# christhetree/mod_extraction

Measured on AMD Instinct MI355X. Metric: 44.1 kHz audio-seconds/sec (train step), interwoven ph/fl/ch, higher is better.
Workload: dtype f32

## Files before the change

mod_extraction_amd/csrc/wgrad_kvec_f16.hip:

```cpp
#include "conv_common.h"
#include <stdlib.h>

typedef _Float16 half8 __attribute__((ext_vector_type(8)));
typedef _Float16 half4 __attribute__((ext_vector_type(4)));
typedef short short4v __attribute__((__vector_size__(4 * sizeof(short))));

#define WK_KS_MAX 6
#define WK_CH (WK_KS_MAX * 32)
#define WK_AP (WK_CH + 16)
#define WK_BR (WK_CH + 12)

#define WK_A_BYTES (2 * 64 * WK_AP * 2)
#define WK_B_ROWS ((WK_BR + 7) / 8 * 8)
#define WK_LDS_BYTES (WK_A_BYTES + 2 * WK_B_ROWS * 32)

struct WgradKvecArgs {
    const float *G;
    const unsigned char *amax;
    const float *scale;
    const _Float16 *xk_hi, *xk_lo;
    float *part;
    int B, H, Wv, rows_per_slab, n_slabs;
    int packed;
};

__device__ __forceinline__ floatx4 mfma_16x16x32(half8 a, half8 b, floatx4 c)
{
    return __builtin_amdgcn_mfma_f32_16x16x32_f16(a, b, c, 0, 0, 0);
}

__device__ __forceinline__ int wk_a_slot(int c8) { return c8 < 4 ? 8 * c8 : 8 * (c8 - 4) + 4; }
__device__ __forceinline__ half8 tr_frag16(const unsigned char *img, int lane_off, int r0)
{
    const unsigned char *ptr = img + lane_off + r0 * 32;
    const short4v v0 = __builtin_amdgcn_ds_read_tr16_b64_v4i16((short4v __attribute__((address_space(3))) *)ptr);
    const short4v v1 = __builtin_amdgcn_ds_read_tr16_b64_v4i16((short4v __attribute__((address_space(3))) *)(ptr + 16 * 32));
    typedef short short8v __attribute__((__vector_size__(8 * sizeof(short))));
    const short8v both = __builtin_shufflevector(v0, v1, 0, 1, 2, 3, 4, 5, 6, 7);
    return __builtin_bit_cast(half8, both);
}

__global__ __launch_bounds__(256, 2) void wgrad_kvec_f16_kernel(WgradKvecArgs a)
{
    extern __shared__ __attribute__((aligned(256))) unsigned char wk_smem[];
    _Float16 *const dzA = reinterpret_cast<_Float16 *>(wk_smem);
    _Float16 *const xB = reinterpret_cast<_Float16 *>(wk_smem + WK_A_BYTES);
    const int tid = threadIdx.x, lane = tid & 63, wave = __builtin_amdgcn_readfirstlane(tid >> 6);
    const int tap0 = wave * 3 + (wave >> 1);
    const int m16 = lane & 15, kg = lane >> 4;
    const int slab = blockIdx.x;
    const int Hp = a.H >> 1;
    const float S = a.scale[0];

    floatx4 acc[CV_KW];
#pragma unroll
    for (int i = 0; i < CV_KW; ++i) acc[i] = floatx4{0.f, 0.f, 0.f, 0.f};

    const int a_lane = (m16 * WK_AP + 8 * kg) * 2;
    const int b_lane = (4 * kg + (m16 >> 2)) * 32 + (m16 & 3) * 8;
    constexpr int A_SPLIT = 64 * WK_AP * 2, B_SPLIT = WK_B_ROWS * 32;
    const unsigned char *Ab = reinterpret_cast<const unsigned char *>(dzA);
    const unsigned char *Bb = reinterpret_cast<const unsigned char *>(xB);

    const int row_begin = slab * a.rows_per_slab;
    int row_end = row_begin + a.rows_per_slab;
    if (row_end > a.B * a.H) row_end = a.B * a.H;
    constexpr int NA = 64 * (WK_CH / 4) / 256, NB = (2 * WK_BR * 2 + 255) / 256;
    floatx4 ga[NA], vb[NB];
    unsigned ama[NA];
    auto issue_g = [&](int rid, int w0) {
        const int b = rid / a.H, h = rid - b * a.H;
        const int npos = (CV_PITCH - w0 >= WK_CH) ? WK_CH : (CV_PITCH - w0);
#pragma unroll
        for (int q = 0; q < NA; ++q) {
            const int i = tid + q * 256, co = i / (WK_CH / 4), c4 = i - co * (WK_CH / 4);
            ga[q] = floatx4{0.f, 0.f, 0.f, 0.f};
            ama[q] = 0x02020202u;
            if (c4 * 4 < npos) {
                const size_t off = (((size_t)b * 64 + co) * Hp + (h >> 1)) * CV_PITCH + w0 + c4 * 4;
                ga[q] = __builtin_nontemporal_load(reinterpret_cast<const floatx4 *>(a.G + off));
                ama[q] = __builtin_nontemporal_load(reinterpret_cast<const unsigned *>(a.amax + off));
            }
        }
    };
    auto issue_x = [&](int rid, int w0) {
        const int b = rid / a.H, h = rid - b * a.H;
        const int npos = (CV_PITCH - w0 >= WK_CH) ? WK_CH : (CV_PITCH - w0);
#pragma unroll
        for (int q = 0; q < NB; ++q) {
            const int i = tid + q * 256;
            const int split = i / (WK_BR * 2), k = i - split * (WK_BR * 2);
            const int pos = k >> 1, part = k & 1, w = w0 - 6 + pos;
            vb[q] = floatx4{0.f, 0.f, 0.f, 0.f};
            if (i < 2 * WK_BR * 2 && pos < npos + 12 && w >= 0 && w < CV_PITCH)
                vb[q] = *reinterpret_cast<const floatx4 *>((split ? a.xk_lo : a.xk_hi) +
                                                           (((size_t)b * a.H + h) * CV_PITCH + w) * 16 + part * 8);
        }
    };
    auto commit = [&](int rid, int w0) {
        const int h = rid % a.H;
        const unsigned want = (unsigned)(h & 1);
#pragma unroll
        for (int q = 0; q < NA; ++q) {
            const int i = tid + q * 256, co = i / (WK_CH / 4), c4 = i - co * (WK_CH / 4);
            const int wq = w0 + c4 * 4;
            half4 hi, lo;
            if (a.packed) {
                unsigned v[4];
#pragma unroll
                for (int e = 0; e < 4; ++e) v[e] = ((ama[q] >> (8 * e)) & 0xffu) == want ? __float_as_uint(ga[q][e]) : 0u;
                const unsigned h01 = __builtin_amdgcn_perm(v[1], v[0], 0x05040100u), h23 = __builtin_amdgcn_perm(v[3], v[2], 0x05040100u);
                const unsigned l01 = __builtin_amdgcn_perm(v[1], v[0], 0x07060302u), l23 = __builtin_amdgcn_perm(v[3], v[2], 0x07060302u);
                typedef unsigned uintx2 __attribute__((ext_vector_type(2)));
                hi = __builtin_bit_cast(half4, uintx2{h01, h23});
                lo = __builtin_bit_cast(half4, uintx2{l01, l23});
            } else {
#pragma unroll
            for (int e = 0; e < 4; ++e) {
                const bool keep = ((ama[q] >> (8 * e)) & 0xffu) == want && wq + e < a.Wv;
                const float v = keep ? ga[q][e] * S : 0.0f;
                const _Float16 hh = (_Float16)v;
                hi[e] = hh;
                lo[e] = (_Float16)(v - (float)hh);
            }
            }
            const int slot = (c4 >> 3) * 32 + wk_a_slot(c4 & 7);
            *reinterpret_cast<half4 *>(dzA + co * WK_AP + slot) = hi;
            *reinterpret_cast<half4 *>(dzA + 64 * WK_AP + co * WK_AP + slot) = lo;
        }
#pragma unroll
        for (int q = 0; q < NB; ++q) {
            const int i = tid + q * 256;
            if (i < 2 * WK_BR * 2) {
                const int split = i / (WK_BR * 2), k = i - split * (WK_BR * 2);
                *reinterpret_cast<floatx4 *>(xB + (size_t)split * (WK_B_ROWS * 16) + (k >> 1) * 16 + (k & 1) * 8) = vb[q];
            }
        }
    };

    int rid = row_begin, w0 = 0;
    if (rid < row_end) { issue_g(rid, w0); issue_x(rid, w0); }
    while (rid < row_end) {
        const int nks = (CV_PITCH - w0 >= WK_CH) ? WK_KS_MAX : (CV_PITCH - w0) / 32;
        int nrid, nw0 = w0;
        if (!(rid & 1)) nrid = rid + 1;
        else {
            nrid = rid - 1;
            nw0 = w0 + WK_CH;
            if (nw0 >= CV_PITCH) { nw0 = 0; nrid = rid + 1; }
        }
        __syncthreads();
        commit(rid, w0);
        if (nrid < row_end) {
            if (!(nrid & 1)) issue_g(nrid, nw0);
            issue_x(nrid, nw0);
        }
        __syncthreads();
        {
            {
#pragma unroll 1
            for (int ks = 0; ks < nks; ++ks) {
                half8 ah[5], al[5], bh[4], bl[4];
#pragma unroll
                for (int j = 0; j < 5; ++j) {
                    const int jt = j < 4 ? j : wave;
                    ah[j] = *reinterpret_cast<const half8 *>(Ab + a_lane + jt * (16 * WK_AP * 2) + ks * 64);
                    al[j] = *reinterpret_cast<const half8 *>(Ab + A_SPLIT + a_lane + jt * (16 * WK_AP * 2) + ks * 64);
                }
#pragma unroll
                for (int t = 0; t < 4; ++t) {
                    const int kw = t < 3 ? tap0 + t : 6;
                    bh[t] = tr_frag16(Bb, b_lane, ks * 32 + kw);
                    bl[t] = tr_frag16(Bb + B_SPLIT, b_lane, ks * 32 + kw);
                }
#pragma unroll
                for (int u = 0; u < 13; ++u) acc[u] = mfma_16x16x32(al[u < 12 ? (u & 3) : 4], bh[u < 12 ? (u >> 2) : 3], acc[u]);
#pragma unroll
                for (int u = 0; u < 13; ++u) acc[u] = mfma_16x16x32(ah[u < 12 ? (u & 3) : 4], bl[u < 12 ? (u >> 2) : 3], acc[u]);
#pragma unroll
                for (int u = 0; u < 13; ++u) acc[u] = mfma_16x16x32(ah[u < 12 ? (u & 3) : 4], bh[u < 12 ? (u >> 2) : 3], acc[u]);
            }
            }
        }
        rid = nrid;
        w0 = nw0;
    }
#pragma unroll
    for (int u = 0; u < CV_KW; ++u) {
        const int kw = u < 12 ? tap0 + (u >> 2) : 6, j = u < 12 ? (u & 3) : wave;
        float *dst = a.part + (((size_t)slab * CV_KW + kw) * 64 + j * 16) * 16;
#pragma unroll
        for (int r = 0; r < 4; ++r) dst[(4 * kg + r) * 16 + m16] = acc[u][r];
    }
}


__global__ __launch_bounds__(256) void wgrad_kvec_reduce_kernel(const float *__restrict__ part, int n_slabs,
                                                                const float *__restrict__ scale, float *__restrict__ dW)
{
    __shared__ double sh[16][17];
    const int total = CV_KW * 64 * 16;
    const int ol = threadIdx.x & 15, sl = threadIdx.x >> 4;
    const int j = blockIdx.x * 16 + ol;
    double s = 0.0;
    for (int i = sl; i < n_slabs; i += 16) s += (double)part[(size_t)i * total + j];
    sh[sl][ol] = s;
    __syncthreads();
    if (sl == 0) {
        double t = 0.0;
#pragma unroll
        for (int q = 0; q < 16; ++q) t += sh[q][ol];
        const int k = j & 15, co = (j >> 4) & 63, kw = j >> 10;
        if (k < 2 * CV_KH) {
            const int kh = k >> 1, ci = k & 1;
            dW[(((size_t)co * 2 + ci) * CV_KH + kh) * CV_KW + kw] = (float)(t * (double)scale[1]);
        }
    }
}

__global__ void wk_pow2_scale_kernel(const unsigned *__restrict__ amax_bits, float *__restrict__ scale)
{
    const float m = __uint_as_float(*amax_bits);
    int e = 0;
    if (m > 0.0f && m < 3.0e38f) {
        frexpf(m, &e);
        e = 10 - e;
        e = e > 100 ? 100 : (e < -100 ? -100 : e);
    }
    scale[0] = ldexpf(1.0f, e);
    scale[1] = ldexpf(1.0f, -e);
}

MX_EXPORT int mx_conv_block1_wgrad_f16(const float *G, const uint8_t *amax, const uint32_t *amax_bits, const void *xk_hi,
                                       const void *xk_lo, int64_t B, int64_t H, int64_t Wv, int64_t rows_per_slab,
                                       float *scale, float *part, float *dW, void *stream)
{
    if (!G || !amax || !amax_bits || !xk_hi || !xk_lo || !scale || !part || !dW || B <= 0 || rows_per_slab <= 0)
        return MX_ERR_ARG;
    if (H < 2 || (H & 1) || Wv <= 0 || Wv > CV_PITCH) return MX_ERR_UNSUPPORTED;
    rows_per_slab += rows_per_slab & 1;
    const int64_t n_slabs = (B * H + rows_per_slab - 1) / rows_per_slab;
    if (n_slabs > 1000000) return MX_ERR_UNSUPPORTED;
    hipStream_t st = (hipStream_t)stream;
    hipLaunchKernelGGL(wk_pow2_scale_kernel, dim3(1), dim3(1), 0, st, amax_bits, scale);
    WgradKvecArgs a{G, amax, scale, (const _Float16 *)xk_hi, (const _Float16 *)xk_lo, part, (int)B, (int)H, (int)Wv,
                    (int)rows_per_slab, (int)n_slabs, 0};
    static MxLdsLatch latch = {};
    if (mx_set_dyn_lds(latch, (const void *)wgrad_kvec_f16_kernel, WK_LDS_BYTES) != MX_OK) return MX_ERR_LAUNCH;
    hipLaunchKernelGGL(wgrad_kvec_f16_kernel, dim3((unsigned)n_slabs), dim3(256), WK_LDS_BYTES, st, a);
    const int total = CV_KW * 64 * 16;
    hipLaunchKernelGGL(wgrad_kvec_reduce_kernel, dim3(total / 16), dim3(256), 0, st, part, (int)n_slabs, scale, dW);
    return mx_launch_status();
}

MX_EXPORT int mx_conv_block1_wgrad_pair_f16(const void *Gp, const uint8_t *amax, const float *scale, const void *xk_hi,
                                            const void *xk_lo, int64_t B, int64_t H, int64_t Wv, int64_t rows_per_slab,
                                            float *part, float *dW, void *stream)
{
    if (!Gp || !amax || !scale || !xk_hi || !xk_lo || !part || !dW || B <= 0 || rows_per_slab <= 0) return MX_ERR_ARG;
    if (H < 2 || (H & 1) || Wv <= 0 || Wv > CV_PITCH) return MX_ERR_UNSUPPORTED;
    rows_per_slab += rows_per_slab & 1;
    const int64_t n_slabs = (B * H + rows_per_slab - 1) / rows_per_slab;
    if (n_slabs > 1000000) return MX_ERR_UNSUPPORTED;
    hipStream_t st = (hipStream_t)stream;
    WgradKvecArgs a{(const float *)Gp, amax, scale, (const _Float16 *)xk_hi, (const _Float16 *)xk_lo, part, (int)B, (int)H, (int)Wv,
                    (int)rows_per_slab, (int)n_slabs, 1};
    static MxLdsLatch latch = {};
    if (mx_set_dyn_lds(latch, (const void *)wgrad_kvec_f16_kernel, WK_LDS_BYTES) != MX_OK) return MX_ERR_LAUNCH;
    hipLaunchKernelGGL(wgrad_kvec_f16_kernel, dim3((unsigned)n_slabs), dim3(256), WK_LDS_BYTES, st, a);
    const int total = CV_KW * 64 * 16;
    hipLaunchKernelGGL(wgrad_kvec_reduce_kernel, dim3(total / 16), dim3(256), 0, st, part, (int)n_slabs, scale, dW);
    return mx_launch_status();
}
```

mod_extraction_amd/models.py:

```python
import logging
import math
import os
from typing import Dict, List, NamedTuple, Optional, Sequence, Tuple

import torch
from torch import Tensor as T, nn

from . import _hip

log = logging.getLogger(__name__)

CONV_PRECISION = os.environ.get("MODEX_CONV_PRECISION", "f16x3")
DEBUG_TAP = None
PITCH = 352
LN_EPS = 1e-5


def htk_mel_filterbank(n_freqs: int, f_min: float, f_max: float, n_mels: int, sample_rate: int) -> T:
    all_freqs = torch.linspace(0, sample_rate // 2, n_freqs)
    m_min = 2595.0 * math.log10(1.0 + (f_min / 700.0))
    m_max = 2595.0 * math.log10(1.0 + (f_max / 700.0))
    m_pts = torch.linspace(m_min, m_max, n_mels + 2)
    f_pts = 700.0 * (10.0 ** (m_pts / 2595.0) - 1.0)
    f_diff = f_pts[1:] - f_pts[:-1]
    slopes = f_pts.unsqueeze(0) - all_freqs.unsqueeze(1)
    down_slopes = (-1.0 * slopes[:, :-2]) / f_diff[:-1]
    up_slopes = slopes[:, 2:] / f_diff[1:]
    return torch.max(torch.zeros(1), torch.min(down_slopes, up_slopes))


def _band_limits(fb: T) -> Tuple[T, T]:
    nz = fb != 0
    any_nz = nz.any(dim=0)
    idx = torch.arange(fb.size(0)).unsqueeze(1).expand_as(fb)
    lo = torch.where(nz, idx, torch.full_like(idx, fb.size(0))).min(dim=0).values
    hi = torch.where(nz, idx + 1, torch.zeros_like(idx)).max(dim=0).values
    lo = torch.where(any_nz, lo, torch.zeros_like(lo))
    return lo.to(torch.int32), hi.to(torch.int32)


class _Buffers(nn.Module):
    """Plain namespace module (gives buffers their torchaudio state-dict key prefixes)."""


class MelSpectrogramHIP(nn.Module):

    def __init__(self, sample_rate: int, n_fft: int, hop_length: int, n_mels: int) -> None:
        super().__init__()
        if n_fft not in (512, 1024, 2048):
            raise NotImplementedError("mx_logmel_fwd is built for n_fft in {512, 1024, 2048}")
        self.sample_rate, self.n_fft, self.hop_length, self.n_mels = sample_rate, n_fft, hop_length, n_mels
        self.spectrogram = _Buffers()
        self.spectrogram.register_buffer("window", torch.hann_window(n_fft))
        self.mel_scale = _Buffers()
        self.mel_scale.register_buffer("fb", htk_mel_filterbank(n_fft // 2 + 1, 0.0, float(sample_rate // 2),
                                                                n_mels, sample_rate))
        k = torch.arange(n_fft, dtype=torch.float64) * (-2.0 * math.pi / n_fft)
        self.register_buffer("twiddle", torch.stack([torch.cos(k), torch.sin(k)], dim=1).float(), persistent=False)
        self._bands: Optional[Tuple[T, T, int]] = None

    def bands(self) -> Tuple[T, T]:
        fb = self.mel_scale.fb
        if self._bands is None or self._bands[2] != fb._version or self._bands[0].device != fb.device:
            lo, hi = _band_limits(fb.detach().cpu())
            self._bands = (lo.to(fb.device), hi.to(fb.device), fb._version)
        return self._bands[0], self._bands[1]

    def log_mel(self, x: T, n_frames: int, eps: float, masks: Sequence[int] = (0, 0, 0, 0), pitch: int = PITCH) -> T:
        B, C, N = x.shape
        xc = x.contiguous().float()
        out = torch.empty((B, C, self.n_mels, pitch), device=x.device, dtype=torch.float32)
        lo, hi = self.bands()
        f0, f1, t0, t1 = (int(v) for v in masks)
        _hip.call("mx_logmel_fwd", _hip.ptr(xc), B * C, N, _hip.ptr(self.spectrogram.window), _hip.ptr(self.twiddle),
                  _hip.ptr(self.mel_scale.fb), _hip.ptr(lo), _hip.ptr(hi), self.n_fft, self.hop_length, self.n_mels,
                  n_frames, pitch, float(eps), f0, f1, t0, t1, _hip.ptr(out), _hip.stream())
        return out


def specaugment_bounds(size: int, mask_param: int) -> Tuple[int, int]:
    value = torch.rand(1) * mask_param
    min_value = torch.rand(1) * (size - value)
    start = int(min_value.long())
    return start, start + int(value.long())


BLOCK1_F16 = os.environ.get("MODEX_BLOCK1", "f16x3") != "f32"
WGRAD_SPARSE = os.environ.get("MODEX_WGRAD", "sparse") != "dense"
WGRAD_SPARSE_MAX_T = int(os.environ.get("MODEX_WGRAD_SP_MAXT", "4"))
DGRAD_SPARSE = os.environ.get("MODEX_DGRAD", "sparse") != "dense"
DIRECT_GRADS = os.environ.get("MODEX_DIRECT_GRADS", "1") != "0"
STATS_FUSED = os.environ.get("MODEX_STATS", "fused") != "sweep"
GPOOL_FUSED = os.environ.get("MODEX_GPOOL", "fused") != "split"
LN_FUSED = os.environ.get("MODEX_LN", "fused") != "sweep"
BLOCK1_PAIR = os.environ.get("MODEX_BLOCK1_PAIR", "1") != "0"

KH, KW, TAPS, CO = 5, 13, 65, 64
W_F16_ELEMS = 4 * KH * KW * CO * 16
W_KVEC_ELEMS = KW * 2 * CO * 8
W_SP_ELEMS = 4 * 3 * 2 * KW * 2 * 64 * 16
KVEC_PART_ELEMS = KW * CO * 16
WS_ROW_KS = 22


def _wgrad_part(n_slabs: int, cin: int, dev) -> T:
    return torch.empty(n_slabs * TAPS * CO * cin, device=dev, dtype=torch.float32)


def _slabs(rows: int, n_target: int) -> Tuple[int, int]:
    rps = max(1, -(-rows // n_target))
    return rps, -(-rows // rps)


def _f16_pair(dev, *shape: int) -> Tuple[T, T]:
    return (torch.empty(shape, device=dev, dtype=torch.float16), torch.empty(shape, device=dev, dtype=torch.float16))


def _f32(dev, *shape: int) -> T:
    return torch.empty(shape, device=dev, dtype=torch.float32)


def _pack(w: T, flip: int) -> T:
    out = _f32(w.device, w.numel())
    _hip.call("mx_conv_pack_weights", _hip.ptr(w.contiguous()), w.size(0), w.size(1), flip, _hip.ptr(out),
              _hip.stream())
    return out


def _pack_f16(w: T, flip: int) -> Tuple[T, T]:
    hi, lo = _f16_pair(w.device, W_F16_ELEMS)
    _hip.call("mx_conv_pack_weights_f16", _hip.ptr(w.contiguous()), flip, _hip.ptr(hi), _hip.ptr(lo), _hip.stream())
    return hi, lo


def _reduce_rows(part: T, rows: int, cols: int, out: Optional[T] = None) -> T:
    if out is None:
        out = _f32(part.device, cols)
    _hip.call("mx_reduce_rows", _hip.ptr(part), rows, cols, 0, _hip.ptr(out), _hip.stream())
    return out


def _direct_grad_views(params) -> Optional[List[T]]:
    views = []
    base = None
    for p in params:
        if not (p.is_leaf and p.requires_grad):
            return None
        g = p.grad
        if g is None or not g.is_contiguous() or g._base is None or g.dtype != torch.float32:
            return None
        if base is None:
            base = g._base
        elif g._base is not base:
            return None
        views.append(g)
    if base is None or not getattr(base, "_modex_fresh", False):
        return None
    base._modex_fresh = False
    return views


class BlockRoute(NamedTuple):
    fwd: str
    stats: str
    leaves_stats: bool
    g_in: str
    operand: Optional[str]
    wgrad: str
    routed_pair: bool
    dgrad: Optional[str]
    ln_bwd: Optional[str]

    @property
    def dgrad_sparse(self) -> bool:
        return self.dgrad in ("sparse", "sparse+ln")


def plan_stack(cin0: int, dilations: Sequence[int], precision: str, n_frames: int,
               operands_kept: bool = True) -> Tuple[BlockRoute, ...]:
    n = len(dilations)
    fits = n_frames <= PITCH - 1
    blocks = []
    for l, t in enumerate(int(t) for t in dilations):
        if precision == "f16x3" and (cin0 if l == 0 else CO) == 64:
            sp_w = WGRAD_SPARSE and t <= WGRAD_SPARSE_MAX_T and fits
            sp_d = DGRAD_SPARSE and fits
            dgrad = ("sparse+ln" if LN_FUSED else "sparse") if sp_d else "dense"
            blocks.append(dict(fwd="f16x3", operand="kept" if operands_kept else "rederived", wgrad="sparse" if sp_w else "dense",
                               routed_pair=not sp_w or (l > 0 and not sp_d), dgrad=dgrad if l > 0 else None))
        elif precision == "f16x3" and l == 0 and cin0 == 2 and BLOCK1_F16 and t == 1:
            blocks.append(dict(fwd="kvec", operand=None, wgrad="f32", routed_pair=False, dgrad=None))
        else:
            blocks.append(dict(fwd="f32", operand=None, wgrad="f32", routed_pair=False, dgrad="f32" if l > 0 else None))
    for l, b in enumerate(blocks):
        b["stats"] = "epilogue" if l > 0 and blocks[l - 1]["leaves_stats"] else "sweep"
        b["leaves_stats"] = STATS_FUSED and l + 1 < n and b["fwd"] != "f32"
    blocks[-1]["g_in"] = "f32+gmax" if blocks[-1]["fwd"] == "f16x3" else "f32"
    kvec_kept = blocks[0]["fwd"] == "kvec" and operands_kept
    for l in range(n - 1, 0, -1):
        b, below = blocks[l], blocks[l - 1]
        pooled_only = l > 1 and below["wgrad"] == "sparse" and below["dgrad"] in ("sparse", "sparse+ln")
        if b["dgrad"] == "sparse+ln" and GPOOL_FUSED and pooled_only:
            b["ln_bwd"], below["g_in"] = "gpool", "pooled"
        elif b["dgrad"] == "sparse+ln" and BLOCK1_PAIR and l == 1 and kvec_kept:
            b["ln_bwd"], below["g_in"] = "pair", "pair"
        elif below["fwd"] == "f16x3" or (l == 1 and kvec_kept):
            b["ln_bwd"], below["g_in"] = "plain+gmax", "f32+gmax"
        else:
            b["ln_bwd"], below["g_in"] = "plain", "f32"
    blocks[0]["ln_bwd"] = None
    if kvec_kept and blocks[0]["g_in"] != "f32":
        blocks[0].update(operand="kept", wgrad="kvec_pair" if blocks[0]["g_in"] == "pair" else "kvec_scaled")
    return tuple(BlockRoute(**b) for b in blocks)


class _Act(NamedTuple):
    p: T
    slope: Optional[T] = None
    bias: Optional[T] = None
    stats_part: Optional[T] = None


class _Grad(NamedTuple):
    G: Optional[T] = None
    gmax: Optional[T] = None
    pooled: Optional[tuple] = None
    pair_scale: Optional[T] = None
    bsum: Optional[T] = None


class _Split(NamedTuple):
    G: Optional[T] = None
    dz: Tuple[Optional[T], Optional[T]] = (None, None)
    gc: Tuple[Optional[T], ...] = (None, None, None)
    scale: Optional[T] = None
    x16: Tuple[Optional[T], Optional[T]] = (None, None)


class _ParamGrads:

    def __init__(self, n: int, direct: Optional[List[T]]) -> None:
        self.direct, self.grads = direct, [None] * n

    def weight(self, i: int, w: T) -> T:
        self.grads[i] = self.direct[i] if self.direct is not None else torch.empty_like(w)
        return self.grads[i]

    def reduce(self, i: int, part: T, rows: int, cols: int) -> None:
        self.grads[i] = _reduce_rows(part, rows, cols, self.direct[i].view(-1) if self.direct is not None else None)

    def for_autograd(self) -> List[Optional[T]]:
        return [None] * len(self.grads) if self.direct is not None else self.grads


def _block_fwd(r: BlockRoute, x: _Act, w: T, b: T, a: T, n_frames: int, t: int, first: bool):
    B, cin, H, _ = x.p.shape
    dev, st = x.p.device, _hip.stream()
    stats = _f32(dev, B, cin, 2)
    if r.stats == "epilogue":
        _hip.call("mx_plane_stats_finish", _hip.ptr(x.stats_part), _hip.ptr(x.bias), _hip.ptr(x.slope), B, cin, H,
                  n_frames, LN_EPS, _hip.ptr(stats), st)
    else:
        _hip.call("mx_plane_stats", _hip.ptr(x.p), _hip.ptr(x.slope), B, cin, H, n_frames, LN_EPS, _hip.ptr(stats), st)
    a_out = a.contiguous()
    p = _f32(dev, B, 64, H // 2, PITCH)
    amax = torch.empty((B, 64, H // 2, PITCH), device=dev, dtype=torch.uint8)
    stats_part = _f32(dev, B, H // 2, 64, 2) if r.leaves_stats else None
    operand = None
    if r.fwd == "f16x3":
        operand = _f16_pair(dev, B, H, 4, PITCH, 16)
        _hip.call("mx_conv_prep_fwd_f16", _hip.ptr(x.p), _hip.ptr(stats), _hip.ptr(x.slope), B, H, n_frames,
                  _hip.ptr(operand[0]), _hip.ptr(operand[1]), st)
        w_hi, w_lo = _pack_f16(w, 0)
        _hip.call("mx_conv_block_fwd_f16", _hip.ptr(operand[0]), _hip.ptr(operand[1]), _hip.ptr(w_hi), _hip.ptr(w_lo),
                  _hip.ptr(b.contiguous()), B, H, n_frames, t, _hip.ptr(p), _hip.ptr(amax),
                  _hip.ptr(a_out) if r.leaves_stats else None, _hip.ptr(stats_part), st)
    elif r.fwd == "kvec":
        operand = _f16_pair(dev, B, H, 1, PITCH, 16)
        _hip.call("mx_conv_prep_fwd_kvec_f16", _hip.ptr(x.p), _hip.ptr(stats), B, H, n_frames, _hip.ptr(operand[0]),
                  _hip.ptr(operand[1]), st)
        wk_hi, wk_lo = _f16_pair(dev, W_KVEC_ELEMS)
        _hip.call("mx_conv_pack_weights_kvec_f16", _hip.ptr(w.detach().contiguous()), _hip.ptr(wk_hi), _hip.ptr(wk_lo), st)
        _hip.call("mx_conv_block1_fwd_f16", _hip.ptr(operand[0]), _hip.ptr(operand[1]), _hip.ptr(wk_hi), _hip.ptr(wk_lo),
                  _hip.ptr(b.contiguous()), B, H, n_frames, _hip.ptr(p), _hip.ptr(amax),
                  _hip.ptr(a_out) if r.leaves_stats else None, _hip.ptr(stats_part), st)
    else:
        wt = _pack(w, 0)
        _hip.call("mx_conv_block_fwd", _hip.ptr(x.p), _hip.ptr(stats), _hip.ptr(x.slope), _hip.ptr(wt),
                  _hip.ptr(b.contiguous()), B, cin, H, n_frames, t, 1 if first else 0, _hip.ptr(p), _hip.ptr(amax), st)
    return _Act(p, a_out, b.contiguous(), stats_part), (x.p, stats, amax), operand


def _head_bwd(r_last: BlockRoute, p_last: T, slope_last: T, wout: T, latent: T, out: T, d_out: T, d_latent: Optional[T],
              n_frames: int, gmax_cell: T, pg: _ParamGrads, i_wout: int, i_slope: int) -> _Grad:
    B, L, Hl, dev = out.size(0), out.size(1), p_last.size(2), out.device
    G = torch.empty_like(p_last)
    dw_part, db_part, ds_part = _f32(dev, B, L * 64), _f32(dev, B, L), _f32(dev, B, 64)
    gmax = gmax_cell if r_last.g_in == "f32+gmax" else None
    _hip.call("mx_head_bwd", _hip.ptr(p_last), _hip.ptr(slope_last), _hip.ptr(wout.contiguous()),
              _hip.ptr(latent), _hip.ptr(out), _hip.ptr(d_out), _hip.ptr(d_latent), B, 64, Hl, n_frames, L,
              _hip.ptr(G), _hip.ptr(dw_part), _hip.ptr(db_part), _hip.ptr(ds_part), _hip.ptr(gmax), _hip.stream())
    pg.reduce(i_wout, dw_part, B, L * 64)
    pg.grads[i_wout] = pg.grads[i_wout].view_as(wout)
    pg.reduce(i_wout + 1, db_part, B, L)
    pg.reduce(i_slope, ds_part, B, 64)
    return _Grad(G=G, gmax=gmax)


def _wgrad_f16x3(r: BlockRoute, l: int, g: _Grad, kept: dict, x_in: T, stats: T, amax: T, slope_prev: Optional[T],
                 n_frames: int, t: int, dW: T) -> _Split:
    B, _, H, _ = x_in.shape
    Hp, dev, st = H // 2, x_in.device, _hip.stream()
    dz = _f16_pair(dev, B, H, 4, PITCH, 16) if r.routed_pair else (None, None)
    if r.g_in == "pooled":
        gc_hi, gc_lo, gc_idx, gidx, scale = g.pooled
    else:
        ready = r.g_in == "f32+gmax"
        ws = g.gmax if ready else torch.empty(1, device=dev, dtype=torch.int32)
        scale = _f32(dev, 2)
        _hip.call("mx_conv_prep_dgrad_f16", _hip.ptr(g.G), _hip.ptr(amax), B, H, n_frames, _hip.ptr(ws),
                  1 if ready else 0, _hip.ptr(scale), _hip.ptr(dz[0]), _hip.ptr(dz[1]), st)
        gc_hi = gc_lo = gc_idx = gidx = None
        if r.wgrad == "sparse" or r.dgrad_sparse:
            gc_hi, gc_lo = _f16_pair(dev, B, Hp, 4, PITCH, 16)
            gc_idx = torch.empty((B, Hp, 4, PITCH), device=dev, dtype=torch.int32)
            if r.wgrad == "sparse":
                gidx = torch.empty((B, 64, Hp, WS_ROW_KS, 2), device=dev, dtype=torch.int16)
            _hip.call("mx_conv_prep_gpool_cl_f16", _hip.ptr(g.G), _hip.ptr(amax), _hip.ptr(scale), B, H, n_frames,
                      _hip.ptr(gc_hi), _hip.ptr(gc_lo), _hip.ptr(gc_idx), _hip.ptr(gidx), st)
    if r.operand == "kept":
        x_hi, x_lo = kept.pop(l)
    else:
        x_hi, x_lo = _f16_pair(dev, B, H, 4, PITCH, 16)
        _hip.call("mx_conv_prep_fwd_f16", _hip.ptr(x_in), _hip.ptr(stats), _hip.ptr(slope_prev), B, H, n_frames,
                  _hip.ptr(x_hi), _hip.ptr(x_lo), st)
    rps, n_slabs = _slabs(B * Hp if r.wgrad == "sparse" else B * H, 256)
    part = _wgrad_part(n_slabs, 64, dev)
    if r.wgrad == "sparse":
        _hip.call("mx_conv_block_wgrad_sp_f16", _hip.ptr(gc_hi), _hip.ptr(gc_lo), _hip.ptr(gidx), _hip.ptr(x_hi),
                  _hip.ptr(x_lo), _hip.ptr(scale), B, H, n_frames, t, rps, _hip.ptr(part), _hip.ptr(dW), st)
    else:
        _hip.call("mx_conv_block_wgrad_f16", _hip.ptr(dz[0]), _hip.ptr(dz[1]), _hip.ptr(x_hi), _hip.ptr(x_lo),
                  _hip.ptr(scale), B, H, t, rps, _hip.ptr(part), _hip.ptr(dW), st)
    return _Split(dz=dz if r.dgrad == "dense" else (None, None), gc=(gc_hi, gc_lo, gc_idx), scale=scale,
                  x16=(x_hi, x_lo) if r.dgrad == "sparse+ln" else (None, None))


def _weight_grad(r: BlockRoute, l: int, g: _Grad, kept: dict, x_in: T, stats: T, amax: T, slope_prev: Optional[T],
                 n_frames: int, t: int, dW: T) -> _Split:
    if r.fwd == "f16x3":
        return _wgrad_f16x3(r, l, g, kept, x_in, stats, amax, slope_prev, n_frames, t, dW)
    B, cin, H, _ = x_in.shape
    dev, st = x_in.device, _hip.stream()
    if r.wgrad in ("kvec_pair", "kvec_scaled"):
        xk_hi, xk_lo = kept.pop(l)
        rps, n_slabs = _slabs(B * H, 2048)
        part = _f32(dev, n_slabs * KVEC_PART_ELEMS)
        if r.wgrad == "kvec_pair":
            _hip.call("mx_conv_block1_wgrad_pair_f16", _hip.ptr(g.G), _hip.ptr(amax), _hip.ptr(g.pair_scale), _hip.ptr(xk_hi),
                      _hip.ptr(xk_lo), B, H, n_frames, rps, _hip.ptr(part), _hip.ptr(dW), st)
        else:
            scale1 = _f32(dev, 2)
            _hip.call("mx_conv_block1_wgrad_f16", _hip.ptr(g.G), _hip.ptr(amax), _hip.ptr(g.gmax), _hip.ptr(xk_hi),
                      _hip.ptr(xk_lo), B, H, n_frames, rps, _hip.ptr(scale1), _hip.ptr(part), _hip.ptr(dW), st)
    else:
        rps, n_slabs = _slabs(B * H, 256 if cin == 64 else 1024)
        part = _wgrad_part(n_slabs, cin, dev)
        _hip.call("mx_conv_block_wgrad", _hip.ptr(g.G), _hip.ptr(amax), _hip.ptr(x_in), _hip.ptr(stats),
                  _hip.ptr(slope_prev), B, cin, H, n_frames, t, rps, _hip.ptr(part), _hip.ptr(dW), st)
    return _Split(G=g.G)


def _data_grad(r: BlockRoute, l: int, d: _Split, w: T, amax: T, B: int, H: int, n_frames: int, t: int, zws: T):
    dev, st = w.device, _hip.stream()
    dxhat = _f32(dev, B, 64, H, PITCH)
    ln_part = gx_bits = None
    if r.dgrad_sparse:
        ws_hi, ws_lo = _f16_pair(dev, W_SP_ELEMS)
        _hip.call("mx_conv_pack_weights_sp_f16", _hip.ptr(w.detach().contiguous()), _hip.ptr(ws_hi), _hip.ptr(ws_lo), st)
        if r.dgrad == "sparse+ln":
            ln_part = _f32(dev, B, 64, H, 2, 2)
            gx_bits = zws[4 * l:4 * l + 2] if r.ln_bwd in ("gpool", "pair") else None
        _hip.call("mx_conv_block_dgrad_sp_f16", _hip.ptr(d.gc[0]), _hip.ptr(d.gc[1]), _hip.ptr(d.gc[2]),
                  _hip.ptr(ws_hi), _hip.ptr(ws_lo), _hip.ptr(d.scale), B, H, n_frames, t,
                  _hip.ptr(dxhat), _hip.ptr(d.x16[0]), _hip.ptr(d.x16[1]), _hip.ptr(ln_part), _hip.ptr(gx_bits), st)
    elif r.dgrad == "dense":
        w_hi, w_lo = _pack_f16(w, 1)
        _hip.call("mx_conv_block_dgrad_f16", _hip.ptr(d.dz[0]), _hip.ptr(d.dz[1]), _hip.ptr(w_hi), _hip.ptr(w_lo),
                  _hip.ptr(d.scale), B, H, n_frames, t, _hip.ptr(dxhat), st)
    else:
        wt_f = _pack(w, 1)
        _hip.call("mx_conv_block_dgrad", _hip.ptr(d.G), _hip.ptr(amax), _hip.ptr(wt_f), B, H, n_frames, t, _hip.ptr(dxhat), st)
    if DEBUG_TAP is not None:
        DEBUG_TAP[f"dxhat{l}"] = dxhat.clone()
    return dxhat, ln_part, gx_bits


def _ln_prelu_bwd(r: BlockRoute, l: int, x_in: T, dxhat: T, ln_part: Optional[T], gx_bits: Optional[T], stats: T,
                  slope_prev: T, amax_below: T, n_frames: int, zws: T) -> Tuple[_Grad, T]:
    B, _, H, _ = x_in.shape
    dev, st = x_in.device, _hip.stream()
    ds_part, bsum = _f32(dev, B, 64), _f32(dev, B, 64)
    if r.ln_bwd in ("gpool", "pair"):
        m12, scale_n = _f32(dev, B, 64, 2), _f32(dev, 2)
        bound_ws = torch.empty(1, device=dev, dtype=torch.int32)
        _hip.call("mx_ln_bwd_finish", _hip.ptr(ln_part), _hip.ptr(stats), _hip.ptr(slope_prev), _hip.ptr(gx_bits),
                  B, 64, H, n_frames, _hip.ptr(m12), _hip.ptr(bound_ws), _hip.ptr(scale_n), st)
    if r.ln_bwd == "gpool":
        gn_hi, gn_lo = _f16_pair(dev, B, H, 4, PITCH, 16)
        gn_idx = torch.empty((B, H, 4, PITCH), device=dev, dtype=torch.int32)
        gn_pidx = torch.empty((B, 64, H, WS_ROW_KS, 2), device=dev, dtype=torch.int16)
        part2 = _f32(dev, B, 64, H, 6, 2)
        _hip.call("mx_ln_prelu_bwd_gpool_f16", _hip.ptr(x_in), _hip.ptr(dxhat), _hip.ptr(amax_below),
                  _hip.ptr(stats), _hip.ptr(slope_prev), _hip.ptr(m12), _hip.ptr(scale_n), B, H, n_frames,
                  _hip.ptr(gn_hi), _hip.ptr(gn_lo), _hip.ptr(gn_idx), _hip.ptr(gn_pidx), _hip.ptr(part2),
                  _hip.ptr(ds_part), _hip.ptr(bsum), st)
        return _Grad(pooled=(gn_hi, gn_lo, gn_idx, gn_pidx, scale_n), bsum=bsum), ds_part
    if r.ln_bwd == "pair":
        _hip.call("mx_ln_prelu_bwd_pair", _hip.ptr(x_in), _hip.ptr(dxhat), _hip.ptr(stats), _hip.ptr(slope_prev),
                  B, 64, H, n_frames, _hip.ptr(ds_part), _hip.ptr(bsum), _hip.ptr(ln_part), _hip.ptr(scale_n), st)
        return _Grad(G=dxhat, pair_scale=scale_n, bsum=bsum), ds_part
    gmax = zws[4 * l + 2:4 * l + 3] if r.ln_bwd == "plain+gmax" else None
    _hip.call("mx_ln_prelu_bwd", _hip.ptr(x_in), _hip.ptr(dxhat), _hip.ptr(stats), _hip.ptr(slope_prev),
              B, 64, H, n_frames, _hip.ptr(ds_part), _hip.ptr(bsum), _hip.ptr(gmax), _hip.ptr(ln_part), st)
    return _Grad(G=dxhat, gmax=gmax, bsum=bsum), ds_part


class _CNNStack(torch.autograd.Function):

    @staticmethod
    def forward(ctx, logmel: T, n_frames: int, dilations: Tuple[int, ...], precision: str, *params: T):
        n_blocks = len(dilations)
        routes = plan_stack(logmel.size(1), dilations, precision, n_frames)
        keep = any(ctx.needs_input_grad)
        ctx.operands = {}
        x, saved = _Act(logmel), []
        for l, r in enumerate(routes):
            x, for_bwd, operand = _block_fwd(r, x, *params[3 * l:3 * l + 3], n_frames, int(dilations[l]), l == 0)
            saved += for_bwd
            if keep and r.operand == "kept":
                ctx.operands[l] = operand
            del operand
        wout, bout = params[3 * n_blocks], params[3 * n_blocks + 1]
        B, H, L, dev = logmel.size(0), x.p.size(2), wout.size(0), logmel.device
        latent, out = _f32(dev, B, 64, n_frames), _f32(dev, B, L, n_frames)
        _hip.call("mx_head_fwd", _hip.ptr(x.p), _hip.ptr(x.slope), _hip.ptr(wout.contiguous()),
                  _hip.ptr(bout.contiguous()), B, 64, H, n_frames, L, _hip.ptr(latent), _hip.ptr(out), _hip.stream())
        ctx.save_for_backward(*saved, x.p, latent, out, *params)
        ctx.param_objs = params
        ctx.meta = (n_frames, tuple(dilations), n_blocks, precision)
        return out, latent

    @staticmethod
    def backward(ctx, d_out: Optional[T], d_latent: Optional[T]):
        n_frames, dilations, n_blocks, precision = ctx.meta
        tensors = ctx.saved_tensors
        saved, (p_last, latent, out), params = tensors[:3 * n_blocks], tensors[3 * n_blocks:3 * n_blocks + 3], \
            tensors[3 * n_blocks + 3:]
        kept, ctx.operands = ctx.operands, None
        routes = plan_stack(saved[0].size(1), dilations, precision, n_frames, operands_kept=kept is not None)
        B, dev = out.size(0), out.device
        pg = _ParamGrads(len(params), _direct_grad_views(ctx.param_objs) if DIRECT_GRADS else None)
        d_out = (d_out if d_out is not None else torch.zeros_like(out)).contiguous()
        d_latent = d_latent.contiguous() if d_latent is not None else None
        zws = torch.zeros(4 * (n_blocks + 1), device=dev, dtype=torch.int32)
        g = _head_bwd(routes[-1], p_last, params[3 * (n_blocks - 1) + 2].contiguous(), params[3 * n_blocks], latent, out,
                      d_out, d_latent, n_frames, zws[4 * n_blocks:4 * n_blocks + 1], pg, 3 * n_blocks, 3 * (n_blocks - 1) + 2)
        for l in range(n_blocks - 1, -1, -1):
            r, t = routes[l], int(dilations[l])
            x_in, stats, amax = saved[3 * l:3 * l + 3]
            H = x_in.size(2)
            slope_prev = params[3 * (l - 1) + 2].contiguous() if l > 0 else None
            if DEBUG_TAP is not None:
                if r.g_in in ("f32", "f32+gmax"):
                    DEBUG_TAP[f"G{l}"] = g.G.clone()
                DEBUG_TAP[f"amax{l}"] = amax.clone()
                DEBUG_TAP[f"p{l}"] = (p_last if l == n_blocks - 1 else saved[3 * (l + 1)]).clone()
            bsum = g.bsum
            if bsum is None:
                bsum = _f32(dev, B, 64)
                _hip.call("mx_plane_sum", _hip.ptr(g.G), B * 64, H // 2, n_frames, _hip.ptr(bsum), _hip.stream())
            pg.reduce(3 * l + 1, bsum, B, 64)
            d = _weight_grad(r, l, g, kept, x_in, stats, amax, slope_prev, n_frames, t, pg.weight(3 * l, params[3 * l]))
            del g, bsum
            if l == 0:
                break
            dxhat, ln_part, gx_bits = _data_grad(r, l, d, params[3 * l], amax, B, H, n_frames, t, zws)
            del d
            g, ds_part = _ln_prelu_bwd(r, l, x_in, dxhat, ln_part, gx_bits, stats, slope_prev, saved[3 * (l - 1) + 2],
                                       n_frames, zws)
            del dxhat, ln_part
            pg.reduce(3 * (l - 1) + 2, ds_part, B, 64)
        return (None, None, None, None, *pg.for_autograd())


class Spectral2DCNN(nn.Module):
    def __init__(self,
                 in_ch: int = 1,
                 n_samples: int = 88200,
                 sr: float = 44100,
                 n_fft: int = 1024,
                 hop_len: int = 256,
                 n_mels: int = 256,
                 kernel_size: Tuple[int, int] = (5, 13),
                 out_channels: Optional[List[int]] = None,
                 bin_dilations: Optional[List[int]] = None,
                 temp_dilations: Optional[List[int]] = None,
                 pool_size: Tuple[int, int] = (3, 1),
                 latent_dim: int = 1,
                 freq_mask_amount: float = 0.0,
                 time_mask_amount: float = 0.0,
                 use_ln: bool = True,
                 eps: float = 1e-7) -> None:
        super().__init__()
        if out_channels is None:
            out_channels = [64] * 5
        if bin_dilations is None:
            bin_dilations = [1] * len(out_channels)
        if temp_dilations is None:
            temp_dilations = [2 ** idx for idx in range(len(out_channels))]
        assert len(out_channels) == len(bin_dilations) == len(temp_dilations)
        assert pool_size[1] == 1
        self.sr, self.n_fft, self.hop_len, self.n_mels = sr, n_fft, hop_len, n_mels
        self.kernel_size, self.pool_size, self.latent_dim = tuple(kernel_size), tuple(pool_size), latent_dim
        self.freq_mask_amount, self.time_mask_amount = freq_mask_amount, time_mask_amount
        self.use_ln, self.eps = use_ln, eps
        self.out_channels, self.bin_dilations, self.temp_dilations = list(out_channels), list(bin_dilations), \
            list(temp_dilations)
        self.in_ch = in_ch
        self.n_frames = n_samples // hop_len + 1
        self.generic = (self.kernel_size != (5, 13) or self.pool_size != (2, 1) or not use_ln
                        or any(c != 64 for c in out_channels) or any(d != 1 for d in bin_dilations)
                        or any(d not in (1, 2, 4, 8, 16) for d in temp_dilations) or in_ch not in (1, 2)
                        or self.n_frames > PITCH or n_mels % (2 ** len(out_channels)) != 0 or latent_dim > 4)
        if self.generic:
            n_bins = n_mels
            for _ in out_channels:
                n_bins //= self.pool_size[0]
            if n_bins < 1 or min(self.kernel_size) < 1 or min(self.bin_dilations + self.temp_dilations) < 1 or self.pool_size[0] > 255:
                raise ValueError(f"Spectral2DCNN: {n_mels} mel bins do not survive {len(out_channels)} poolings by "
                                 f"{self.pool_size[0]} (or a kernel size / dilation below 1)")
        self.conv_precision = CONV_PRECISION
        self.spectrogram = MelSpectrogramHIP(int(sr), n_fft, hop_len, n_mels)
        self.freq_mask_param = int(freq_mask_amount * n_mels)
        self.time_mask_param = int(time_mask_amount * self.n_frames)
        layers: List[nn.Module] = []
        n_bins, c_in = n_mels, in_ch
        for out_ch, b_dil, t_dil in zip(out_channels, bin_dilations, temp_dilations):
            if use_ln:
                layers.append(nn.LayerNorm([n_bins, self.n_frames], elementwise_affine=False))
            layers.append(nn.Conv2d(c_in, out_ch, self.kernel_size, stride=(1, 1), dilation=(b_dil, t_dil),
                                    padding="same"))
            layers.append(nn.MaxPool2d(kernel_size=self.pool_size))
            layers.append(nn.PReLU(num_parameters=out_ch))
            c_in, n_bins = out_ch, n_bins // self.pool_size[0]
        self.cnn = nn.Sequential(*layers)
        self.output = nn.Conv1d(out_channels[-1], latent_dim, kernel_size=(1,))

    def _stack_params(self) -> List[T]:
        ps: List[T] = []
        per, first = (4, 1) if self.use_ln else (3, 0)
        for i in range(len(self.out_channels)):
            conv, prelu = self.cnn[per * i + first], self.cnn[per * i + first + 2]
            w = conv.weight
            if i == 0 and self.in_ch == 1 and not self.generic:
                w = torch.cat([w, torch.zeros_like(w)], dim=1)
            ps += [w, conv.bias, prelu.weight]
        ps += [self.output.weight, self.output.bias]
        return ps

    def draw_masks(self) -> Tuple[int, int, int, int]:
        f0 = f1 = t0 = t1 = 0
        if self.training:
            if self.freq_mask_amount > 0:
                f0, f1 = specaugment_bounds(self.n_mels, self.freq_mask_param)
            if self.time_mask_amount > 0:
                t0, t1 = specaugment_bounds(self.n_frames, self.time_mask_param)
        return f0, f1, t0, t1

    def log_mel(self, x: T, masks: Optional[Sequence[int]] = None) -> T:
        assert x.ndim == 3
        n_frames = x.size(-1) // self.hop_len + 1
        assert n_frames == self.n_frames, "clip length does not match the LayerNorm shape"
        masks = self.draw_masks() if masks is None else masks
        if self.generic:
            with torch.no_grad():
                return self.spectrogram.log_mel(x, self.n_frames, self.eps, masks, pitch=self.n_frames)
        if self.in_ch == 1:
            x = torch.cat([x, torch.zeros_like(x)], dim=1)
        with torch.no_grad():
            return self.spectrogram.log_mel(x, self.n_frames, self.eps, masks)

    def forward(self, x: T, masks: Optional[Sequence[int]] = None) -> (T, T):
        logmel = self.log_mel(x, masks)
        if self.generic:
            from .cnn_generic import GenericCNNStack
            cfg = (self.kernel_size, int(self.pool_size[0]), bool(self.use_ln),
                   tuple(zip(self.out_channels, self.bin_dilations, self.temp_dilations)))
            return GenericCNNStack.apply(logmel, cfg, *self._stack_params())
        out, latent = _CNNStack.apply(logmel, self.n_frames, tuple(self.temp_dilations), self.conv_precision,
                                      *self._stack_params())
        return out, latent


class RandomLFO(nn.Module):

    def __init__(self,
                 n_samples: int,
                 sr: float,
                 use_shape_gt: bool = False,
                 use_phase_gt: bool = False,
                 use_freq_gt: bool = False,
                 shapes: Optional[List[str]] = None,
                 freq_min: float = 0.5,
                 freq_max: float = 3.0,
                 phase_error: float = 0.0,
                 freq_error: float = 0.0) -> None:
        super().__init__()
        self.n_samples, self.sr = n_samples, sr
        self.use_shape_gt, self.use_phase_gt, self.use_freq_gt = use_shape_gt, use_phase_gt, use_freq_gt
        self.shapes, self.freq_min, self.freq_max = shapes, freq_min, freq_max
        self.phase_error, self.freq_error = phase_error, freq_error

    def forward(self, batch_size: int, fx_params: Optional[Dict[str, T]] = None) -> T:
        from .modulations import make_rand_mod_signal
        shapes_gt = phase_gt = freq_gt = None
        if self.use_shape_gt:
            assert fx_params is not None and "shape" in fx_params
            shapes_gt = fx_params["shape"]
        if self.use_phase_gt:
            assert fx_params is not None and "phase" in fx_params
            phase_gt = fx_params["phase"]
        if self.use_freq_gt:
            assert fx_params is not None and "rate_hz" in fx_params
            freq_gt = fx_params["rate_hz"]
        return make_rand_mod_signal(batch_size, self.n_samples, self.sr, self.freq_min, self.freq_max, shapes_gt,
                                    self.shapes, phase_gt, self.phase_error, freq_gt, self.freq_error).unsqueeze(1)


class SpectrogramHIP(nn.Module):

    def __init__(self, n_fft: int, hop_length: int) -> None:
        super().__init__()
        if n_fft not in (512, 1024, 2048):
            raise NotImplementedError("mx_logmel_fwd is built for n_fft in {512, 1024, 2048}")
        self.n_fft, self.hop_length, self.n_bins = n_fft, hop_length, n_fft // 2 + 1
        self.register_buffer("window", torch.hann_window(n_fft))
        k = torch.arange(n_fft, dtype=torch.float64) * (-2.0 * math.pi / n_fft)
        self.register_buffer("twiddle", torch.stack([torch.cos(k), torch.sin(k)], dim=1).float(), persistent=False)
        self.register_buffer("eye", torch.eye(self.n_bins), persistent=False)
        self.register_buffer("band_lo", torch.arange(self.n_bins, dtype=torch.int32), persistent=False)
        self.register_buffer("band_hi", torch.arange(1, self.n_bins + 1, dtype=torch.int32), persistent=False)

    def log_power(self, x: T, n_frames: int, eps: float) -> T:
        assert x.ndim == 3 and x.size(1) == 1
        B, _, N = x.shape
        xc = x.contiguous().float()
        out = torch.empty((B, self.n_bins, PITCH), device=x.device, dtype=torch.float32)
        _hip.call("mx_logmel_fwd", _hip.ptr(xc), B, N, _hip.ptr(self.window), _hip.ptr(self.twiddle), _hip.ptr(self.eye),
                  _hip.ptr(self.band_lo), _hip.ptr(self.band_hi), self.n_fft, self.hop_length, self.n_bins, n_frames, PITCH,
                  float(eps), 0, 0, 0, 0, _hip.ptr(out), _hip.stream())
        return out

# ... 227 lines not shown
```

Before: 7635.

## Add 2:4 structured-sparse SMFMAC kernel for block-1 paired weight gradient

Adds a new block-1 weight-gradient kernel that exploits the 2:4 sparsity pattern implied by max-pool amax indices. It packs the pooled gradient into compressed halves plus nibble indices in LDS and uses smfmac 16x16x64 instructions, halving the MFMA work and reading the pooled G directly. The host signals sparse vs dense via the parity of rows_per_slab, which is an opaque encoding, and the new kernel uses a smaller channel chunk and different LDS layout.

```diff
diff --git a/mod_extraction_amd/csrc/wgrad_kvec_f16.hip b/mod_extraction_amd/csrc/wgrad_kvec_f16.hip
--- a/mod_extraction_amd/csrc/wgrad_kvec_f16.hip
+++ b/mod_extraction_amd/csrc/wgrad_kvec_f16.hip
@@ -180,6 +180,175 @@
 #pragma unroll
                 for (int u = 0; u < 13; ++u) acc[u] = mfma_16x16x32(ah[u < 12 ? (u & 3) : 4], bh[u < 12 ? (u >> 2) : 3], acc[u]);
             }
+            }
+        }
+        rid = nrid;
+        w0 = nw0;
+    }
+#pragma unroll
+    for (int u = 0; u < CV_KW; ++u) {
+        const int kw = u < 12 ? tap0 + (u >> 2) : 6, j = u < 12 ? (u & 3) : wave;
+        float *dst = a.part + (((size_t)slab * CV_KW + kw) * 64 + j * 16) * 16;
+#pragma unroll
+        for (int r = 0; r < 4; ++r) dst[(4 * kg + r) * 16 + m16] = acc[u][r];
+    }
+}
+
+typedef _Float16 half16 __attribute__((ext_vector_type(16)));
+#define WS_KS 4
+#define WS_CH (WS_KS * 32)
+#define WS_AP (WS_CH + 16)
+#define WS_BR (WS_CH + 12)
+#define WS_BROWS (WS_BR + 2)
+#define WS_BPAR (WS_BROWS * 32)
+#define WS_BSPLIT (2 * WS_BPAR)
+#define WS_A_BYTES (2 * 64 * WS_AP * 2)
+#define WS_LDS_BYTES (WS_A_BYTES + 2 * WS_BSPLIT)
+#define WS_IX_OFF (WS_CH * 2)
+
+__device__ __forceinline__ half16 tr_frag_sp(const unsigned char *img, int lane_off, int r0)
+{
+    typedef short4v __attribute__((address_space(3))) * lds4;
+    const unsigned char *ptr = img + lane_off + r0 * 32;
+    const short4v v0 = __builtin_amdgcn_ds_read_tr16_b64_v4i16((lds4)ptr);
+    const short4v v1 = __builtin_amdgcn_ds_read_tr16_b64_v4i16((lds4)(ptr + 2 * 32));
+    const short4v v2 = __builtin_amdgcn_ds_read_tr16_b64_v4i16((lds4)(ptr + 16 * 32));
+    const short4v v3 = __builtin_amdgcn_ds_read_tr16_b64_v4i16((lds4)(ptr + 18 * 32));
+    typedef short short8v __attribute__((__vector_size__(8 * sizeof(short))));
+    typedef short short16v __attribute__((__vector_size__(16 * sizeof(short))));
+    const short8v a = __builtin_shufflevector(v0, v1, 0, 1, 2, 3, 4, 5, 6, 7), b = __builtin_shufflevector(v2, v3, 0, 1, 2, 3, 4, 5, 6, 7);
+    const short16v all = __builtin_shufflevector(a, b, 0, 1, 2, 3, 4, 5, 6, 7, 8, 9, 10, 11, 12, 13, 14, 15);
+    return __builtin_bit_cast(half16, all);
+}
+
+__global__ __launch_bounds__(256, 2) void wgrad_kvec_sp_f16_kernel(WgradKvecArgs a)
+{
+    extern __shared__ __attribute__((aligned(256))) unsigned char wk_smem[];
+    _Float16 *const dzA = reinterpret_cast<_Float16 *>(wk_smem);
+    unsigned char *const xB = wk_smem + WS_A_BYTES;
+    const int tid = threadIdx.x, lane = tid & 63, wave = __builtin_amdgcn_readfirstlane(tid >> 6);
+    const int tap0 = wave * 3 + (wave >> 1);
+    const int m16 = lane & 15, kg = lane >> 4;
+    const int slab = blockIdx.x;
+    const int Hp = a.H >> 1;
+
+    floatx4 acc[CV_KW];
+#pragma unroll
+    for (int i = 0; i < CV_KW; ++i) acc[i] = floatx4{0.f, 0.f, 0.f, 0.f};
+
+    constexpr int A_SPLIT = 64 * WS_AP * 2, A_TILE = 16 * WS_AP * 2;
+    const int a_lane = (m16 * WS_AP + 8 * kg) * 2;
+    const int i_lane = m16 * WS_AP * 2 + WS_IX_OFF + 2 * kg;
+    const int b_lane = ((m16 >> 3) & 1) * WS_BPAR + (4 * kg + ((m16 >> 2) & 1)) * 32 + (m16 & 3) * 8;
+    const unsigned char *Ab = reinterpret_cast<const unsigned char *>(dzA);
+    const unsigned char *Bb = xB;
+
+    const int row_begin = slab * a.rows_per_slab;
+    int row_end = row_begin + a.rows_per_slab;
+    if (row_end > a.B * a.H) row_end = a.B * a.H;
+    constexpr int NA = 64 * (WS_CH / 4) / 256, NB = 5;
+    static_assert(WS_BR * 2 == 256 + 24, "the B staging deals 256 + 24 items per image");
+    const int t_par = lane >= 24, t_k = 256 + lane - 24 * t_par;
+    floatx4 vb[NB];
+    typedef unsigned uintx4 __attribute__((ext_vector_type(4)));
+    uintx4 ga[NA];
+    unsigned ama[NA];
+    auto issue = [&](int rid, int w0) {
+        const int b = rid / a.H, h = rid - b * a.H;
+        const int npos = (CV_PITCH - w0 >= WS_CH) ? WS_CH : (CV_PITCH - w0);
+#pragma unroll
+        for (int q = 0; q < NA; ++q) {
+            const int i = tid + q * 256, co = i / (WS_CH / 4), c4 = i - co * (WS_CH / 4);
+            ga[q] = uintx4{0u, 0u, 0u, 0u};
+            ama[q] = 0x02020202u;
+            if (c4 * 4 < npos) {
+                const size_t off = (((size_t)b * 64 + co) * Hp + (h >> 1)) * CV_PITCH + w0 + c4 * 4;
+                ga[q] = __builtin_nontemporal_load(reinterpret_cast<const uintx4 *>(a.G + off));
+                ama[q] = __builtin_nontemporal_load(reinterpret_cast<const unsigned *>(a.amax + off));
+            }
+        }
+        const long xoff = (((long)b * a.H + h) * CV_PITCH + w0 - 6) * 16;
+#pragma unroll
+        for (int img = 0; img < 4; ++img) {
+            const _Float16 *src = ((img >> 1) ? a.xk_lo : a.xk_hi) + xoff + (img & 1) * (CV_PITCH * 16);
+            const int pos = tid >> 1, w = w0 - 6 + pos;
+            vb[img] = floatx4{0.f, 0.f, 0.f, 0.f};
+            if (pos < npos + 12 && w >= 0 && w < CV_PITCH) vb[img] = *reinterpret_cast<const floatx4 *>(src + tid * 8);
+        }
+        vb[4] = floatx4{0.f, 0.f, 0.f, 0.f};
+        if (wave < 2 && lane < 48) {
+            const _Float16 *src = (wave ? a.xk_lo : a.xk_hi) + xoff + t_par * (CV_PITCH * 16);
+            const int pos = t_k >> 1, w = w0 - 6 + pos;
+            if (pos < npos + 12 && w >= 0 && w < CV_PITCH) vb[4] = *reinterpret_cast<const floatx4 *>(src + t_k * 8);
+        }
+    };
+    auto commit = [&]() {
+#pragma unroll
+        for (int q = 0; q < NA; ++q) {
+            const int i = tid + q * 256, co = i / (WS_CH / 4), c4 = i - co * (WS_CH / 4);
+            unsigned first[2], second[2], nib = 0;
+#pragma unroll
+            for (int c = 0; c < 2; ++c) {
+                const unsigned a0 = (ama[q] >> (16 * c)) & 0xffu, a1 = (ama[q] >> (16 * c + 8)) & 0xffu;
+                const unsigned x0 = a0 < 2u ? ga[q][2 * c] : 0u, x1 = a1 < 2u ? ga[q][2 * c + 1] : 0u;
+                const unsigned sel = (a0 & 1u) + 2u * (a1 & 1u);
+                const bool swap = sel == 1u;
+                first[c] = swap ? x1 : x0;
+                second[c] = swap ? x0 : x1;
+                nib |= ((0xEC94u >> (4 * sel)) & 0xfu) << (4 * c);
+            }
+            const unsigned h01 = __builtin_amdgcn_perm(second[0], first[0], 0x05040100u), h23 = __builtin_amdgcn_perm(second[1], first[1], 0x05040100u);
+            const unsigned l01 = __builtin_amdgcn_perm(second[0], first[0], 0x07060302u), l23 = __builtin_amdgcn_perm(second[1], first[1], 0x07060302u);
+            typedef unsigned uintx2 __attribute__((ext_vector_type(2)));
+            *reinterpret_cast<uintx2 *>(dzA + co * WS_AP + c4 * 4) = uintx2{h01, h23};
+            *reinterpret_cast<uintx2 *>(dzA + 64 * WS_AP + co * WS_AP + c4 * 4) = uintx2{l01, l23};
+            wk_smem[co * WS_AP * 2 + WS_IX_OFF + c4] = (unsigned char)nib;
+        }
+#pragma unroll
+        for (int img = 0; img < 4; ++img) *reinterpret_cast<floatx4 *>(xB + img * WS_BPAR + tid * 16) = vb[img];
+        if (wave < 2 && lane < 48) *reinterpret_cast<floatx4 *>(xB + (wave * 2 + t_par) * WS_BPAR + t_k * 16) = vb[4];
+    };
+
+    int rid = row_begin, w0 = 0;
+    if (rid < row_end) issue(rid, w0);
+    while (rid < row_end) {
+        const int nks = (CV_PITCH - w0 >= WS_CH) ? WS_KS : (CV_PITCH - w0) / 32;
+        int nrid = rid, nw0 = w0 + WS_CH;
+        if (nw0 >= CV_PITCH) { nw0 = 0; nrid = rid + 2; }
+        __syncthreads();
+        commit();
+        if (nrid < row_end) issue(nrid, nw0);
+        __syncthreads();
+#pragma unroll 1
+        for (int ks = 0; ks < nks; ++ks) {
+            half8 ah[5], al[5];
+            int ix[5];
+#pragma unroll
+            for (int j = 0; j < 4; ++j) {
+                const int jt = j;
+                ah[j] = *reinterpret_cast<const half8 *>(Ab + a_lane + jt * A_TILE + ks * 64);
+                al[j] = *reinterpret_cast<const half8 *>(Ab + A_SPLIT + a_lane + jt * A_TILE + ks * 64);
+                ix[j] = *reinterpret_cast<const unsigned short *>(Ab + i_lane + jt * A_TILE + ks * 8);
+            }
+#pragma unroll
+            for (int t = 0; t < 4; ++t) {
+                const int kw = t < 3 ? tap0 + t : 6;
+                const half16 bh = tr_frag_sp(Bb, b_lane, ks * 32 + kw), bl = tr_frag_sp(Bb + WS_BSPLIT, b_lane, ks * 32 + kw);
+                const int nj = t < 3 ? 4 : 1;
+                if (t == 3) {
+                    ah[4] = *reinterpret_cast<const half8 *>(Ab + a_lane + wave * A_TILE + ks * 64);
+                    al[4] = *reinterpret_cast<const half8 *>(Ab + A_SPLIT + a_lane + wave * A_TILE + ks * 64);
+                    ix[4] = *reinterpret_cast<const unsigned short *>(Ab + i_lane + wave * A_TILE + ks * 8);
+                }
+#pragma unroll
+                for (int pass = 0; pass < 3; ++pass) {
+                    const int pr = pass == 2 ? 2 : 1 - pass;
+#pragma unroll
+                    for (int j = 0; j < nj; ++j) {
+                        const int u = t < 3 ? 4 * t + j : 12, f = t < 3 ? j : 4;
+                        acc[u] = __builtin_amdgcn_smfmac_f32_16x16x64_f16(pr == 0 ? al[f] : ah[f], pr == 1 ? bl : bh, acc[u], ix[f], 0, 0);
+                    }
+                }
             }
         }
         rid = nrid;
@@ -259,15 +428,21 @@
 {
     if (!Gp || !amax || !scale || !xk_hi || !xk_lo || !part || !dW || B <= 0 || rows_per_slab <= 0) return MX_ERR_ARG;
     if (H < 2 || (H & 1) || Wv <= 0 || Wv > CV_PITCH) return MX_ERR_UNSUPPORTED;
+    const bool sparse = !(rows_per_slab & 1);
     rows_per_slab += rows_per_slab & 1;
     const int64_t n_slabs = (B * H + rows_per_slab - 1) / rows_per_slab;
     if (n_slabs > 1000000) return MX_ERR_UNSUPPORTED;
     hipStream_t st = (hipStream_t)stream;
     WgradKvecArgs a{(const float *)Gp, amax, scale, (const _Float16 *)xk_hi, (const _Float16 *)xk_lo, part, (int)B, (int)H, (int)Wv,
                     (int)rows_per_slab, (int)n_slabs, 1};
-    static MxLdsLatch latch = {};
-    if (mx_set_dyn_lds(latch, (const void *)wgrad_kvec_f16_kernel, WK_LDS_BYTES) != MX_OK) return MX_ERR_LAUNCH;
-    hipLaunchKernelGGL(wgrad_kvec_f16_kernel, dim3((unsigned)n_slabs), dim3(256), WK_LDS_BYTES, st, a);
+    static MxLdsLatch latch = {}, latch_sp = {};
+    if (sparse) {
+        if (mx_set_dyn_lds(latch_sp, (const void *)wgrad_kvec_sp_f16_kernel, WS_LDS_BYTES) != MX_OK) return MX_ERR_LAUNCH;
+        hipLaunchKernelGGL(wgrad_kvec_sp_f16_kernel, dim3((unsigned)n_slabs), dim3(256), WS_LDS_BYTES, st, a);
+    } else {
+        if (mx_set_dyn_lds(latch, (const void *)wgrad_kvec_f16_kernel, WK_LDS_BYTES) != MX_OK) return MX_ERR_LAUNCH;
+        hipLaunchKernelGGL(wgrad_kvec_f16_kernel, dim3((unsigned)n_slabs), dim3(256), WK_LDS_BYTES, st, a);
+    }
     const int total = CV_KW * 64 * 16;
     hipLaunchKernelGGL(wgrad_kvec_reduce_kernel, dim3(total / 16), dim3(256), 0, st, part, (int)n_slabs, scale, dW);
     return mx_launch_status();
diff --git a/mod_extraction_amd/models.py b/mod_extraction_amd/models.py
--- a/mod_extraction_amd/models.py
+++ b/mod_extraction_amd/models.py
@@ -94,6 +94,7 @@
 GPOOL_FUSED = os.environ.get("MODEX_GPOOL", "fused") != "split"
 LN_FUSED = os.environ.get("MODEX_LN", "fused") != "sweep"
 BLOCK1_PAIR = os.environ.get("MODEX_BLOCK1_PAIR", "1") != "0"
+BLOCK1_WGRAD_SPARSE = True
 
 KH, KW, TAPS, CO = 5, 13, 65, 64
 W_F16_ELEMS = 4 * KH * KW * CO * 16
@@ -210,7 +211,8 @@
             b["ln_bwd"], below["g_in"] = "plain", "f32"
     blocks[0]["ln_bwd"] = None
     if kvec_kept and blocks[0]["g_in"] != "f32":
-        blocks[0].update(operand="kept", wgrad="kvec_pair" if blocks[0]["g_in"] == "pair" else "kvec_scaled")
+        pair = "kvec_pair" if BLOCK1_WGRAD_SPARSE else "kvec_pair_dense"
+        blocks[0].update(operand="kept", wgrad=pair if blocks[0]["g_in"] == "pair" else "kvec_scaled")
     return tuple(BlockRoute(**b) for b in blocks)
 
 
@@ -352,13 +354,14 @@
         return _wgrad_f16x3(r, l, g, kept, x_in, stats, amax, slope_prev, n_frames, t, dW)
     B, cin, H, _ = x_in.shape
     dev, st = x_in.device, _hip.stream()
-    if r.wgrad in ("kvec_pair", "kvec_scaled"):
+    if r.wgrad in ("kvec_pair", "kvec_pair_dense", "kvec_scaled"):
         xk_hi, xk_lo = kept.pop(l)
         rps, n_slabs = _slabs(B * H, 2048)
         part = _f32(dev, n_slabs * KVEC_PART_ELEMS)
-        if r.wgrad == "kvec_pair":
+        if r.wgrad != "kvec_scaled":
+            rps += rps & 1
             _hip.call("mx_conv_block1_wgrad_pair_f16", _hip.ptr(g.G), _hip.ptr(amax), _hip.ptr(g.pair_scale), _hip.ptr(xk_hi),
-                      _hip.ptr(xk_lo), B, H, n_frames, rps, _hip.ptr(part), _hip.ptr(dW), st)
+                      _hip.ptr(xk_lo), B, H, n_frames, rps if r.wgrad == "kvec_pair" else rps - 1, _hip.ptr(part), _hip.ptr(dW), st)
         else:
             scale1 = _f32(dev, 2)
             _hip.call("mx_conv_block1_wgrad_f16", _hip.ptr(g.G), _hip.ptr(amax), _hip.ptr(g.gmax), _hip.ptr(xk_hi),
```

Result: no change. 7657 (median of 6 runs) (+0.3%).
